# dtarb/TauDEM

Measured on AMD Instinct MI355X. Metric: Mcells/s (PitRemove->D8FlowDir->AreaD8 pipeline), higher is better.
Workload: dtype f32

## Files before the change

### taudem_amd/csrc/flats.hpp

```cpp
#pragma once
#include <algorithm>
#include <functional>
#include <vector>

#include "context.hpp"
#include "device_common.hpp"
#include "strips.hpp"
#include "tile_relax.hpp"

struct FlatLevels { int T; int Tr; int has_pits; };
struct FlatPhases { const char *classify, *levels, *stats, *directions, *next; };
static inline const FlatPhases& flat_phases(int iteration) {
    static const FlatPhases P[4] = {{"flats 1: classify", "flats 1: level fields", "flats 1: statistics", "flats 1: directions", "flats 1: next elev"},
                                    {"flats 2: classify", "flats 2: level fields", "flats 2: statistics", "flats 2: directions", "flats 2: next elev"},
                                    {"flats 3: classify", "flats 3: level fields", "flats 3: statistics", "flats 3: directions", "flats 3: next elev"},
                                    {"flats 4+: classify", "flats 4+: level fields", "flats 4+: statistics", "flats 4+: directions", "flats 4+: next elev"}};
    return P[iteration < 1 ? 0 : (iteration > 4 ? 3 : iteration - 1)];
}
using lvl_t = int16_t;
constexpr int LVL_SAT = 32767;
constexpr int TDX_FLATS_TOO_DEEP = -4242;
template <class LV>
struct FlatBuffersT { LV* lvl; LV* rq; };
using FlatBuffers = FlatBuffersT<lvl_t>;
// ... 291 lines not shown
    static __device__ __forceinline__ bool raw_can_move(S g) { return g >= 0; }
    __device__ __forceinline__ void store(size_t idx, int v) const { G[idx] = S(v); }
    __device__ __forceinline__ uint8_t cell_raw(size_t idx) const { return M[idx]; }
    static __device__ __forceinline__ void cell_decode(uint8_t m, int& cst, unsigned& mask) { cst = 0; mask = m; }
    static __device__ __forceinline__ int apply(int, int own, int m) {
        int t = m + INC;
        if (sizeof(S) == 2 && INC) t = unsigned(t - LVL_SAT) < unsigned(inf() - LVL_SAT) ? LVL_SAT : t;
        return t < own ? t : own;
    }
    static __device__ __forceinline__ int cell_floor(int cst, int) { return cst; }
    static __device__ __forceinline__ bool settled(int, int v) { return v <= 1; }
    static __device__ __forceinline__ int act_never() { return int(0x80000000u); }
    static __device__ __forceinline__ int act_threshold(uint8_t m, int v) { return m ? v - INC : act_never(); }
    static __device__ __forceinline__ int act_threshold_raw(S g) { return g >= 0 ? decode(g) - INC : act_never(); }

    __device__ __forceinline__ int macro_update(const tilek::TileGeom& g, int tile, int k, int* __restrict__ lds, tilek::TileLds& TL, uint32_t* __restrict__ flags_next,
                                                unsigned long long* __restrict__ dbg = nullptr) const {
        const int tid = int(threadIdx.x);
        const unsigned long long tq0 = dbg ? __builtin_readcyclecounter() : 0ull;
        const int W = k * tilek::TS, L = W + 2;
        const int tx0 = tile % g.tiles_x, ty0 = tile / g.tiles_x;
        const int X0 = tx0 * tilek::TS, Y0 = ty0 * tilek::TS;
        const size_t pitch = size_t(g.nx);
        int* const h = lds; int* const pre = h + MACRO_LMAX; int* const suf = pre + MACRO_LMAX; int* const pm = suf + MACRO_LMAX; int* const sp = pm + MACRO_LMAX;
        int* const acc = sp + MACRO_LMAX;
        int* const moved = acc + 4 * (MACRO_LMAX - 2);
        constexpr int AW = MACRO_LMAX - 2;
        if (tid < 8) moved[tid] = 0;
        __syncthreads();
        auto rim_idx = [&](int e, int i) -> size_t {
            const int x = e == 2 ? 0 : (e == 3 ? W - 1 : i), y = e == 0 ? 0 : (e == 1 ? W - 1 : i);
// ... 126 lines not shown
                    for (int i = j - 2; i <= j; i++) if (i >= 0 && i < W && chg[E * AW + i] < best) best = chg[E * AW + i];
                    gain = best + INC < decode(raw_ring[E][u]);
                }
                const int p = j == 0 ? -1 : (j - 1) / tilek::TS;
                const int p0 = __builtin_amdgcn_readfirstlane(p);
                const unsigned long long b_lo = __ballot(gain && p == p0), b_hi = __ballot(gain && p != p0);
                if ((tid & 63) == 0) {
                    if (b_lo != 0ull) atomicOr(&moved[E], 1 << (p0 + 1));
                    if (b_hi != 0ull) atomicOr(&moved[E], 1 << (p0 + 2));
                }
            }
        __syncthreads();
        const unsigned long long tq2 = dbg ? __builtin_readcyclecounter() : 0ull;
        if (tid < 4 * (k + 2)) {
            const int e = tid / (k + 2), j = tid % (k + 2) - 1;
            if (((moved[e] >> (j + 1)) & 1) && out_target >= 0) {
                if (atomicMax(&flags_next[tilek::entry_tile(uint32_t(out_target))], tilek::FLAG_HALO) == 0u) TL.pend[atomicAdd(&TL.npend, 1u)] = uint32_t(out_target);
            }
        }
        __syncthreads();
        if (dbg && tid == 0) {
            const unsigned long long tq3 = __builtin_readcyclecounter();
            atomicAdd(dbg + 9, tq1 - tq0); atomicAdd(dbg + 10, tq2 - tq1); atomicAdd(dbg + 11, tq3 - tq2);
        }
        return 0;
    }
};
using LevelOp = LevelOpT<1, lvl_t>;
using ReachOp = LevelOpT<0, int32_t>;

template <class LV>
static __global__ __launch_bounds__(256) void flat_stats_kernel(const uint32_t* __restrict__ list, unsigned long long nq,
                                                                const LV* __restrict__ lvl, const LV* __restrict__ rq,
// ... 292 lines not shown
    Op op{field, mask};
    if constexpr (Op::kHasPlain) op.TM = tile_masked;
    for (;;) {
        bool left = false;
        int rc = (st.multi() && eager_rounds > 0) ? tile_relax_run_bounded(ctx, op, geom, sc, eager_rounds, &left, rounds, launches) : tile_relax_run(ctx, op, geom, sc, rounds, launches);
        if (rc != TDX_OK) return rc;
        if (!st.multi()) return TDX_OK;
        int64_t changed = 0;
        rc = strip_exchange<typename Op::Raw>(ctx, st, field, typename Op::Raw(-1), sc.flags, geom.tiles_x, &changed, true, left ? 1 : 0);
        if (rc != TDX_OK) return rc;
        if (changed == 0) return TDX_OK;
    }
}

using StreamClassifyFn = std::function<void(const tilek::TileGeom&, uint8_t* fmask, uint8_t* rmask, uint32_t* tile_flags, uint8_t* tile_masked, uint8_t* notfull)>;
template <class Traits, class LV>
static int flats_bfs(tdx_context* ctx, Traits tr, const float* Z, const Strip& st, const uint32_t* qlist, unsigned long long nq,
                     FlatBuffersT<LV> b, FlatLevels* out, tdx_stats* stats, const StreamClassifyFn* stream_classify = nullptr, int iteration = 1) {
    using LOp = flatk::LevelOpT<1, LV>;
    const FlatPhases& ph = flat_phases(iteration);
    ctx->phase = ph.classify;
    hipStream_t s = ctx->stream;
    const int nx = st.nx;
    const size_t n = size_t(nx) * size_t(st.ny_arr);
    const tilek::TileGeom geom = tilek::make_geom(nx, st.ny_arr, st.y0, st.y1);
    const int ntiles = geom.tiles_x * geom.tiles_y;
    unsigned long long* d_cnt = reinterpret_cast<unsigned long long*>(ctx->d_mail);
    uint8_t* fmask = static_cast<uint8_t*>(ctx->scratch(TDX_S_E, n));
    uint8_t* rmask = static_cast<uint8_t*>(ctx->scratch(TDX_S_F, n));
    uint32_t* flags0 = static_cast<uint32_t*>(ctx->scratch(TDX_S_G, size_t(ntiles) * 4 * 2 + size_t(ntiles)));
// ... 49 lines not shown
    if (macro_k) {
        const int y_lo = st.multi() ? st.y0 + 1 : st.y0, y_hi = st.multi() ? st.y1 - 1 : st.y1;
        const unsigned nreg = unsigned(((geom.tiles_x + 7) / 8) * ((geom.tiles_y + 7) / 8));
        hipLaunchKernelGGL(flatk::find_blocks_kernel, dim3((nreg + 63) / 64, 2), dim3(64), 0, s, notfull, geom.tiles_x, geom.tiles_y, nx, y_lo, y_hi, macro_k, remapF, blkF, remapR, blkR);
        geomF.remap = remapF; geomF.blk_k = blkF;
        geomR.remap = remapR; geomR.blk_k = blkR;
    }
    if (pair) {
        uint32_t* listB = flagsB + ntiles;
        const bool two_streams = getenv("TDX_FLATS_FUSED") == nullptr || getenv("TDX_RELAX_LDS") != nullptr;
        const uint32_t* start_flags = two_streams ? flags0 : nullptr;
        if (!two_streams) {
            TDX_HIP_CHECK(ctx, hipMemcpyAsync(flags, flags0, size_t(ntiles) * 4, hipMemcpyDeviceToDevice, s));
            TDX_HIP_CHECK(ctx, hipMemcpyAsync(flagsB, flags0, size_t(ntiles) * 4, hipMemcpyDeviceToDevice, s));
        }
        for (;;) {
            rc = two_streams ? tile_relax_run_pair(ctx, LOp{b.lvl, fmask, tmask}, tilek::Sched{flags, list, counts},
                                                   LOp{b.rq, rmask, no_plain ? tmask : nullptr}, tilek::Sched{flagsB, listB, countsB}, geomF, &rounds_fall, &launches, start_flags, &geomR)
                             : tile_relax_run_fused(ctx, LOp{b.lvl, fmask, tmask}, tilek::Sched{flags, list, counts},
                                                    LOp{b.rq, rmask, no_plain ? tmask : nullptr}, tilek::Sched{flagsB, listB, countsB}, geom, &rounds_fall, &launches);
            if (rc != TDX_OK) return rc;
            start_flags = nullptr;
            if (!st.multi()) break;
            int64_t ch_fall = 0, ch_rise = 0;
            rc = strip_exchange<LV>(ctx, st, b.lvl, LV(-1), flags, geom.tiles_x, &ch_fall);
            if (rc != TDX_OK) return rc;
            rc = strip_exchange<LV>(ctx, st, b.rq, LV(-1), flagsB, geom.tiles_x, &ch_rise);
            if (rc != TDX_OK) return rc;
            int64_t changed = ch_fall + ch_rise;
            rc = strip_allreduce(ctx, st, &changed, 1, TDX_OP_SUM);
            if (rc != TDX_OK) return rc;
            if (changed == 0) break;
        }
    } else {
        const unsigned cg = tdx_blocks_for(size_t(ntiles), 256);
        TDX_HIP_CHECK(ctx, hipMemcpyAsync(flags, flags0, size_t(ntiles) * 4, hipMemcpyDeviceToDevice, s));
        if (macro_k) hipLaunchKernelGGL(flatk::block_flags_kernel, dim3(cg), dim3(256), 0, s, flags, remapF, ntiles);
// ... 61 lines not shown
```

### taudem_amd/csrc/pitremove.hip

```cpp
#include "context.hpp"
#include "device_common.hpp"
#include "strips.hpp"
#include "tile_relax.hpp"

namespace {

constexpr int SEED_ROWS = 16;
constexpr int SEED_CF = 8;
template <int MODE>
__global__ __launch_bounds__(256) void pit_seed_kernel(const float* __restrict__ Z, const int16_t* __restrict__ mask,
                                                       float* __restrict__ W, int nx, int ny, int y_own0, int y_own1, float nodata, int step,
                                                       float* __restrict__ Zc, float* __restrict__ Wc, int nxc, int nyc, int nbx, int xmap) {
    const int bx = tdxk::xcd_block_x(nbx, xmap);
    if (bx < 0) return;
    const int x = bx * 64 + (threadIdx.x & 63);
    const int ybase = y_own0 + blockIdx.y * (4 * SEED_ROWS) + (threadIdx.x >> 6) * SEED_ROWS;
    const bool colok = x < nx;
    const int xc = colok ? x : nx - 1, xm = xc > 0 ? xc - 1 : xc, xp = xc < nx - 1 ? xc + 1 : xc;
    const int lane = int(threadIdx.x & 63);
    const bool edge_lane = lane == 0 || lane == 63;
    const int xe = lane == 0 ? xm : xp;
    float zm[SEED_ROWS + 2], zedge[SEED_ROWS + 2];
#pragma unroll
    for (int j = 0; j < SEED_ROWS + 2; j++) {
// ... 189 lines not shown
};

}

static int pit_finish_level(tdx_context* ctx, const Strip& ls, float* Zc, float* Wc, int nxc, int nyc, int64_t cells_all, tilek::Sched sc, int depth,
                            int64_t* rounds, int64_t* launches, int64_t* own_rounds = nullptr);

static inline Strip pit_level_strip(const Strip& st, int nxc, int nyc) {
    Strip ls;
    ls.nx = nxc; ls.comm = st.comm;
    if (st.multi()) { ls.ny_arr = nyc + 2; ls.y0 = 1; ls.y1 = nyc + 1; ls.up = st.up; ls.down = st.down; }
    else { ls.ny_arr = nyc; ls.y0 = 0; ls.y1 = nyc; }
    return ls;
}

template <int NBR>
static int pit_relax_level(tdx_context* ctx, const Strip& ls, const float* Z, float* W, tilek::Sched sc, int64_t* rounds, int64_t* launches, int64_t* outer,
                           bool all_tiles = true) {
    const tilek::TileGeom g = tilek::make_geom(ls.nx, ls.ny_arr, ls.y0, ls.y1);
    for (;;) {
        int rc = tile_relax_run(ctx, PitOp<NBR>{Z, W}, g, sc, rounds, launches, all_tiles);
        all_tiles = false;
        if (rc != TDX_OK) return rc;
        if (outer) (*outer)++;
        if (!ls.multi()) break;
        int64_t changed = 0;
        rc = strip_exchange<float>(ctx, ls, W, TDX_FEL_NODATA, sc.flags, g.tiles_x, &changed, true);
        if (rc != TDX_OK) return rc;
        if (changed == 0) break;
    }
    return TDX_OK;
}

static int pit_coarse_start(tdx_context* ctx, const Strip& st, const float* Z, float* W, int nx, int nyo, int64_t cells_all, tilek::Sched sc, int depth,
                            int64_t* rounds, int64_t* launches) {
    if (depth >= 3 || cells_all < (int64_t(1) << 18) || nyo < 1) return TDX_OK;
// ... 76 lines not shown
            hipLaunchKernelGGL(pit_seed_kernel<2>, sgrid, dim3(256), 0, s, d_dem, d_mask, d_fel, st.nx, st.ny_arr, st.y0, st.y1, dem_nodata, 1, Zc + off, Wc + off, nxc, nyc, sbx, sxmap);
            if (stats) stats->launches[TDX_K_STENCIL]++;
        }
    } else {
        TdxSpan sp(ctx, TDX_K_STENCIL);
        hipLaunchKernelGGL(pit_seed_kernel<0>, sgrid, dim3(256), 0, s, d_dem, d_mask, d_fel, st.nx, st.ny_arr, st.y0, st.y1, dem_nodata, fourway ? 2 : 1,
                           static_cast<float*>(nullptr), static_cast<float*>(nullptr), 0, 0, sbx, sxmap);
        if (stats) stats->launches[TDX_K_STENCIL]++;
    }
    ctx->phase = "fine level";
    rc = strip_exchange<float>(ctx, st, d_fel, TDX_FEL_NODATA);
    if (rc != TDX_OK) return rc;
    {
        TdxSpan sp(ctx, TDX_K_RELAX);
        bool all_tiles = true;
        const int vc_env = getenv("TDX_PIT_VCYCLE_AFTER") ? std::max(0, atoi(getenv("TDX_PIT_VCYCLE_AFTER"))) : 8;
        if (used_coarse && vc_env > 0) {
            bool left = false;
            rc = tile_relax_run_bounded(ctx, PitOp<8>{d_dem, d_fel}, geom, sched, vc_env, &left, &rounds, &launches, true);
            if (rc != TDX_OK) return rc;
            all_tiles = false;
            const int vc_min = getenv("TDX_PIT_VCYCLE_MIN") ? atoi(getenv("TDX_PIT_VCYCLE_MIN")) : 16;
            if (st.multi() || (left && level1_rounds >= vc_min)) {
                const int nxc = (st.nx + CF - 1) / CF, nyc = (nyo + CF - 1) / CF;
                const Strip ls = pit_level_strip(st, nxc, nyc);
                const size_t off = size_t(ls.y0) * size_t(nxc);
                float* Zc = static_cast<float*>(ctx->scratch(TDX_S_D, size_t(nxc) * size_t(ls.ny_arr) * 4));
                float* Wc = static_cast<float*>(ctx->scratch(TDX_S_E, size_t(nxc) * size_t(ls.ny_arr) * 4));
                const tilek::TileGeom gc = tilek::make_geom(ls.nx, ls.ny_arr, ls.y0, ls.y1);
                const size_t ntc = size_t(gc.tiles_x) * size_t(gc.tiles_y);
                uint32_t* cflags = static_cast<uint32_t*>(ctx->scratch(TDX_S_L, ntc * 4 * (1 + tilek::SCHED_LIST_WORDS)));
                unsigned long long* ccounts = static_cast<unsigned long long*>(ctx->scratch(TDX_S_M, size_t(tilek::COUNT_RING) * 16));
                float* Ur = static_cast<float*>(ctx->scratch(TDX_S_N, size_t(nxc) * size_t(nyc) * 4));
                if (!Zc || !Wc || !cflags || !ccounts || !Ur) return TDX_ERR_NOMEM;
// ... 6 lines not shown
                    rc = strip_exchange<float>(ctx, ls, Wc, TDX_FEL_NODATA, cflags, gc.tiles_x, &changed);
                    if (rc != TDX_OK) return rc;
                }
                rc = pit_relax_level<8>(ctx, ls, Zc, Wc, tilek::Sched{cflags, cflags + ntc, ccounts}, &rounds, &launches, nullptr, false);
                if (rc != TDX_OK) return rc;
                hipLaunchKernelGGL(pit_prolong_min_kernel, dim3((st.nx + 63) / 64, (nyc + 3) / 4), dim3(256), 0, s, d_fel + size_t(st.y0) * size_t(st.nx), st.nx, nyo, Wc + off, Ur, nxc, nyc,
                                   st.y0, st.ny_arr, geom.tiles_x, flags);
                ctx->phase = "fine level";
                if (st.multi()) {
                    int64_t changed = 0;
                    rc = strip_exchange<float>(ctx, st, d_fel, TDX_FEL_NODATA, flags, geom.tiles_x, &changed);
                    if (rc != TDX_OK) return rc;
                }
            }
        }
        rc = fourway ? pit_relax_level<4>(ctx, st, d_dem, d_fel, sched, &rounds, &launches, &outer, all_tiles) : pit_relax_level<8>(ctx, st, d_dem, d_fel, sched, &rounds, &launches, &outer, all_tiles);
        if (rc != TDX_OK) return rc;
        if (stats) stats->launches[TDX_K_RELAX] += launches;
    }
    TDX_HIP_CHECK(ctx, hipGetLastError());
    if (stats) { stats->rounds = rounds; stats->cells_evaluated = outer; }
    ctx->end_call();
    return TDX_OK;
}

static int pitremove_check(tdx_context* ctx, const void* dem, const void* fel, int64_t nx, int64_t ny, int64_t halo, const char* who) {
    if (!ctx || !dem || !fel || nx <= 0 || ny <= 0) return tdx_fail(ctx, TDX_ERR_ARG, who);
    return too_big(nx, ny + halo) ? tdx_fail(ctx, TDX_ERR_ARG, "raster larger than 2^32 cells per device strip") : TDX_OK;
}

extern "C" int tdx_pitremove_dev(tdx_context* ctx, const float* d_dem, int64_t nx, int64_t ny, float dem_nodata,
// ... 22 lines not shown
```

### taudem_amd/csrc/tile_relax.hpp

```cpp
#pragma once
#include <atomic>
#include <algorithm>
#include <chrono>
#include <cstdlib>
#include <functional>
#include <type_traits>

#include "context.hpp"
#include "device_common.hpp"

namespace tilek {
using namespace tdxk;

constexpr int TS = 64;
constexpr int LH = TS + 2;
constexpr int LP = LH + 1;
constexpr int RPW = 16;
constexpr int NWAVE = TS / RPW;
constexpr int NTHR = NWAVE * 64;
constexpr int COUNT_RING = 1024;
constexpr int MAX_SWEEPS = 8;
constexpr int PULL_MAX = 64;
constexpr unsigned MACRO_DEAL_MAX = 4096;
constexpr unsigned MACRO_WGS_MIN = MACRO_DEAL_MAX / PULL_MAX;
// ... 58 lines not shown


__device__ __forceinline__ unsigned mask_at(const unsigned (&pk)[RPW / 4], int r) { return (pk[r >> 2] >> (8 * (r & 3))) & 0xFFu; }

struct TileLds {
    int rim;
    unsigned long long top[2][NWAVE], bot[2][NWAVE];
    unsigned any[2][NWAVE];
    unsigned rows[NWAVE];
    unsigned next;
    unsigned long long base;
    unsigned npend;
    int chain;
    uint32_t pulled[PULL_MAX];
    uint32_t pend[PULL_MAX * 9];
};

constexpr uint32_t FLAG_HALO = 1u, FLAG_FULL = 2u;
constexpr uint32_t TILE_IDX_MASK = 0x07ffffffu;
constexpr int TILE_BLK_SHIFT = 27;
__device__ __forceinline__ int entry_tile(uint32_t e) { return int(e & TILE_IDX_MASK); }
__device__ __forceinline__ int entry_blk_k(uint32_t e) { const unsigned c = (e >> TILE_BLK_SHIFT) & 3u; return c ? 1 << c : 0; }

__device__ __forceinline__ void activate_tiles_around(int x, int y, int nx, int ny, int tiles_x, uint32_t* __restrict__ tile_flags) {
#pragma unroll
    for (int dy = -1; dy <= 1; dy++)
#pragma unroll
        for (int dx = -1; dx <= 1; dx++) {
            const int xn = x + dx, yn = y + dy;
            if (xn >= 0 && xn < nx && yn >= 0 && yn < ny) tile_flags[(yn / TS) * tiles_x + xn / TS] = FLAG_FULL;
// ... 644 lines not shown
                    if (threadIdx.x == 0 && (bal == 0ull || (bal & (bal - 1ull)) != 0ull)) L.chain = -1;
                }
                __builtin_amdgcn_fence(__ATOMIC_SEQ_CST, "agent");
                __syncthreads();
                const int ch = L.chain;
                if (ch == -1) break;
                if (entry_blk_k(uint32_t(ch))) break;
                tile = entry_tile(uint32_t(ch));
                full = ch < 0;
            }
            if (res & (RES_CHANGED | RES_CAPPED)) flag_neighbours(res, tile, g, flags_next, L);
        }
    }
}

template <class Op, class = void>
struct relax_waves : std::integral_constant<int, 4> {};
template <class Op>
struct relax_waves<Op, std::void_t<decltype(Op::kWaves)>> : std::integral_constant<int, Op::kWaves> {};
template <class Body>
__device__ __forceinline__ void round_driver(const uint32_t* __restrict__ list, unsigned long long* __restrict__ count, uint32_t* __restrict__ flags_cur,
                                             uint32_t* __restrict__ flags_next, uint32_t* __restrict__ list_next, unsigned pull_max, const TileGeom& g,
                                             TileLds& L, Body body) {
    round_driver(list, count, flags_cur, flags_next, list_next, pull_max, g, L, body, blockIdx.x, gridDim.x);
}

template <class Op, class = void>
struct has_plain : std::false_type {};
template <class Op>
struct has_plain<Op, std::enable_if_t<Op::kHasPlain>> : std::true_type {};

template <class Op, class = void>
struct has_macro : std::false_type {};
template <class Op>
struct has_macro<Op, std::enable_if_t<(Op::kMacroLdsWords > 0)>> : std::true_type {};
template <class Op, bool = has_macro<Op>::value>
struct macro_lds_words : std::integral_constant<int, 0> {};
template <class Op>
struct macro_lds_words<Op, true> : std::integral_constant<int, Op::kMacroLdsWords> {};

template <class Op>
__device__ __forceinline__ void macro_role(const Op& op, const TileGeom& g, const uint32_t* __restrict__ list, unsigned long long* __restrict__ count,
                                           uint32_t* __restrict__ flags_next, uint32_t* __restrict__ list_next, int* __restrict__ lds, TileLds& L, unsigned bid, unsigned nblocks,
                                           unsigned long long* __restrict__ dbg) {
    const unsigned nact = unsigned(count[0]);
    if (threadIdx.x == 0) L.npend = 0u;
    auto serve = [&](unsigned nb) {
        for (unsigned b = 0; b < nb; b++) {
            const int tile = entry_tile(L.pulled[b]), kb = entry_blk_k(L.pulled[b]);
            const unsigned long long tc0 = dbg ? __builtin_readcyclecounter() : 0ull;
            (void)op.macro_update(g, tile, kb, lds, L, flags_next, dbg);
            if (dbg && threadIdx.x == 0) { atomicAdd(dbg + 13, __builtin_readcyclecounter() - tc0); atomicAdd(dbg + 14, 1ull); }
            const unsigned npend = L.npend;
            if (threadIdx.x == 0) L.base = npend ? atomicAdd(count + 1, (unsigned long long)npend) : 0ull;
            __syncthreads();
            const unsigned long long lb = L.base;
            for (unsigned q = threadIdx.x; q < npend; q += blockDim.x) list_next[lb + q] = L.pend[q];
            __syncthreads();
            if (threadIdx.x == 0) L.npend = 0u;
        }
    };
    if (nact <= MACRO_DEAL_MAX) {
        constexpr int PER = 16;
        static_assert(PER * NTHR == MACRO_DEAL_MAX, "every entry of a dealt round is looked at");
        uint32_t ent[PER];
        unsigned kk[PER];
        const unsigned first = threadIdx.x * PER;
        (void)first;
#pragma unroll
        for (int j = 0; j < PER; j++) { const unsigned i = unsigned(j) * NTHR + threadIdx.x; ent[j] = i < nact ? list[i] : 0u; }
        unsigned mine = 0;
#pragma unroll
        for (int j = 0; j < PER; j++) { kk[j] = unsigned(entry_blk_k(ent[j])); mine += kk[j] != 0u; }
        unsigned incl = mine;
// ... 32 lines not shown
        serve(nb);
    }
}

template <class Op, bool REG>
__global__ __launch_bounds__(NTHR, relax_waves<Op>::value) void relax_kernel(Op op, TileGeom g, const uint32_t* __restrict__ list, unsigned long long* __restrict__ count,
                                                    uint32_t* __restrict__ flags_cur, uint32_t* __restrict__ flags_next,
                                                    uint32_t* __restrict__ list_next, unsigned pull_max, unsigned long long* __restrict__ dbg, unsigned grid_tiles) {
    using T = typename Op::T;
    static_assert(sizeof(T) == 4, "tile engine works on 4-byte values");
    constexpr int kLdsWords = REG ? (REG_LDS_WORDS > macro_lds_words<Op>::value ? REG_LDS_WORDS : macro_lds_words<Op>::value) : LH * LP;
    __shared__ T sV[kLdsWords];
    __shared__ TileLds L;
    if constexpr (REG && has_macro<Op>::value) {
        if (grid_tiles != 0u && blockIdx.x >= grid_tiles) {
            macro_role(op, g, list, count, flags_next, list_next, reinterpret_cast<int*>(sV), L, blockIdx.x - grid_tiles, gridDim.x - grid_tiles, dbg);
            return;
        }
    }
    const unsigned nblocks = grid_tiles != 0u ? grid_tiles : gridDim.x;
    round_driver(list, count, flags_cur, flags_next, list_next, pull_max, g, L, [&](int tile, bool full) {
        if constexpr (REG && has_plain<Op>::value) {
            if (!__builtin_amdgcn_readfirstlane(int(op.tile_masked(tile)))) return relax_tile_reg(op.plain(), g, tile, sV, L, dbg);
        }
        return REG ? relax_tile_reg(op, g, tile, sV, L, dbg) : relax_tile(op, g, tile, full, sV, L, dbg);
    }, blockIdx.x, nblocks);
}

struct RoundArgs { const uint32_t* list; unsigned long long* count; uint32_t* flags_cur; uint32_t* flags_next; uint32_t* list_next; };
template <class Op>
__global__ __launch_bounds__(NTHR, relax_waves<Op>::value) void relax_pair_kernel(Op opA, Op opB, TileGeom g, RoundArgs a, RoundArgs b, unsigned gridA,
                                                                                  unsigned pull_max) {
    using T = typename Op::T;
    static_assert(sizeof(T) == 4, "tile engine works on 4-byte values");
    __shared__ T sV[REG_LDS_WORDS];
    __shared__ TileLds L;
    const bool second = blockIdx.x >= gridA;
    const Op op = second ? opB : opA;
    const RoundArgs ra = second ? b : a;
    round_driver(ra.list, ra.count, ra.flags_cur, ra.flags_next, ra.list_next, pull_max, g, L,
                 [&](int tile, bool) {
// ... 147 lines not shown
    const int t = blockIdx.x * 256 + threadIdx.x;
    const uint32_t f = t < ntiles ? flags0[t] : 0u;
    const uint32_t ra = (remapA != nullptr && t < ntiles) ? remapA[t] : uint32_t(t), rb = (remapB != nullptr && t < ntiles) ? remapB[t] : uint32_t(t);
    const uint32_t fa = entry_tile(ra) != t ? 0u : f, fb = entry_tile(rb) != t ? 0u : f;
    if (t < ntiles) { flagsA[t] = fa; flagsB[t] = fb; flagsA1[t] = 0u; flagsB1[t] = 0u; }
    const unsigned long long pa = block_reserve(fa != 0u ? 1u : 0u, countA);
    if (fa != 0u) listA[pa] = ra;
    const unsigned long long pb = block_reserve(fb != 0u ? 1u : 0u, countB);
    if (fb != 0u) listB[pb] = rb;
}
static __global__ __launch_bounds__(256) void all_start_kernel(int ntiles, uint32_t* __restrict__ flags, uint32_t* __restrict__ flags1, uint32_t* __restrict__ list,
                                                               unsigned long long* __restrict__ counts) {
    const int t = blockIdx.x * 256 + threadIdx.x;
    if (t < ntiles) { flags[t] = FLAG_FULL; flags1[t] = 0u; list[t] = uint32_t(t); }
    if (t < 2 * COUNT_RING) counts[t] = t == 0 ? (unsigned long long)ntiles : 0ull;
}

static __global__ __launch_bounds__(256) void ring_wrap_kernel(unsigned long long* __restrict__ counts, int r) {
    const unsigned long long pending = counts[r];
    __syncthreads();
    for (int i = threadIdx.x; i < 2 * COUNT_RING; i += 256) counts[i] = 0ull;
    __syncthreads();
    if (threadIdx.x == 0) counts[0] = pending;
}

static __global__ __launch_bounds__(256) void flags_fold_kernel(uint32_t* __restrict__ f_first, uint32_t* __restrict__ f_second, int ntiles) {
    const int t = blockIdx.x * 256 + threadIdx.x;
    if (t >= ntiles) return;
    const uint32_t b = f_second[t];
    if (b) { f_second[t] = 0u; if (b > f_first[t]) f_first[t] = b; }
// ... 42 lines not shown
    const unsigned err = unsigned(host_mail[3] & 0xffffffffull);
    *gave_up = err != 0;
    if (err) {
        fprintf(stderr, "taudem_amd: asynchronous tile worklist gave up (code %u, head %llu tail %llu pending %d); continuing with the round schedule\n", err,
                (unsigned long long)host_mail[0], (unsigned long long)host_mail[1], int(host_mail[2] & 0xffffffffull));
        hipLaunchKernelGGL(fill_u32_kernel, dim3(cgrid), dim3(256), 0, s, sc.flags, FLAG_FULL, size_t(ntiles));
    }
    return TDX_OK;
}

template <class Op>
struct RoundRunner {
    tdx_context* ctx; hipStream_t s; Op op; tilek::TileGeom g; tilek::Sched sc; uint64_t* h; unsigned long long* dbg;
    int ntiles; unsigned cgrid, grid_full, grid_small;
    bool print_counts = false;
    int ring_len;
    bool lds_variant;
    unsigned pull_max;
    int r = 0, parity = 0, batch = 4;
    int r_enq = 0, parity_enq = 0, n_enq = 0, n_col = 0, fl_batch[2] = {0, 0};
    bool polled[2] = {false, false};
    uint64_t fl_tag[2] = {0, 0};
    int ev_base = 0;
    int batch_max = 64;
    bool done = false;
    int64_t rounds = 0, launches = 0;
    bool short_tail = getenv("TDX_RELAX_LONG_TAIL") == nullptr;
    unsigned long long last_count = 0;
    std::function<void(const tilek::TileGeom& rg, unsigned grid, hipStream_t st, const uint32_t* list, unsigned long long* count, uint32_t* flags_cur,
                       uint32_t* flags_next, uint32_t* list_next, unsigned pull_max)> custom_launch;
    RoundRunner(tdx_context* c, hipStream_t st, Op o, tilek::TileGeom geom, tilek::Sched sched, uint64_t* host_mail, unsigned long long* d)
        : ctx(c), s(st), op(o), g(geom), sc(sched), h(host_mail), dbg(d) {
        ntiles = g.tiles_x * g.tiles_y;
        cgrid = tdx_blocks_for(size_t(ntiles), 256);
        grid_full = unsigned(std::min(ntiles, 8 * ctx->num_cus));
        static const int gs_env = getenv("TDX_RELAX_GRID_SMALL") ? std::max(1, atoi(getenv("TDX_RELAX_GRID_SMALL"))) : 0;
        grid_small = unsigned(std::min(ntiles, gs_env ? gs_env : ctx->num_cus));
        const char* e = getenv("TDX_RELAX_RING");
        ring_len = e ? std::max(3, std::min(atoi(e), tilek::COUNT_RING)) : tilek::COUNT_RING;
        lds_variant = getenv("TDX_RELAX_LDS") != nullptr;
        const char* pm = getenv("TDX_RELAX_PULL");
        pull_max = pm ? unsigned(std::max(1, std::min(atoi(pm), tilek::PULL_MAX))) : 16u;
    }
    uint32_t* list_of(int p) const { return sc.list + size_t(p) * size_t(ntiles); }
    uint32_t* flags_of(int p) const { return p ? sc.list + 2 * size_t(ntiles) : sc.flags; }
    bool prestarted = false;
    bool all_tiles = false;
    int start() {
        using namespace tilek;
        r = 0; parity = 0;
        r_enq = 0; parity_enq = 0; n_enq = 0; n_col = 0;
        if (prestarted) return TDX_OK;
        if (all_tiles) {
            hipLaunchKernelGGL(all_start_kernel, dim3(tdx_blocks_for(size_t(std::max(ntiles, 2 * COUNT_RING)), 256)), dim3(256), 0, s, ntiles, sc.flags, flags_of(1), list_of(0), sc.counts);
            return TDX_OK;
        }
        TDX_HIP_CHECK(ctx, hipMemsetAsync(sc.counts, 0, size_t(2 * COUNT_RING) * sizeof(unsigned long long), s));
        TDX_HIP_CHECK(ctx, hipMemsetAsync(flags_of(1), 0, size_t(ntiles) * 4, s));
        hipLaunchKernelGGL(first_list_kernel, dim3(cgrid), dim3(256), 0, s, sc.flags, ntiles, list_of(0), sc.counts, g.remap);
        r = 0; parity = 0;
        r_enq = 0; parity_enq = 0; n_enq = 0; n_col = 0;
        return TDX_OK;
    }
// ... 78 lines not shown
                    return tdx_fail(ctx, TDX_ERR_HIP, "tile schedule: no report from a batch of rounds after " + std::to_string(int(limit_s)) + " s");
            }
            __builtin_ia32_pause();
        }
        std::atomic_thread_fence(std::memory_order_acquire);
        return TDX_OK;
    }
    void collect() {
        const int slot = n_col & 1, nb = fl_batch[slot];
        const volatile uint64_t* hs = h + slot * TDX_MAIL_RUN_SLOT;
        for (int b = 0; b < nb; b++) {
            const uint64_t cnt = polled[slot] ? (hs[b] & 0xffffffffull) : hs[b];
            if (cnt == 0) { done = true; break; }
            last_count = cnt;
            rounds++;
            if (print_counts) fprintf(stderr, " %llu", (unsigned long long)cnt);
        }
        r += nb;
        parity = (parity + nb) & 1;
        n_col++;
    }
    static int pipelined_batch_max() {
        static const int v = getenv("TDX_RELAX_BATCH") ? std::max(2, std::min(atoi(getenv("TDX_RELAX_BATCH")), 64)) : 16;
        return v;
    }
    int drive() {
        batch_max = pipelined_batch_max();
        int rc = start();
        if (rc != TDX_OK) return rc;
        rc = enqueue();
        if (rc != TDX_OK) return rc;
// ... 62 lines not shown
    while (!A.done || !B.done) {
        rc = enqueue_fused(A, B);
        if (rc != TDX_OK) return rc;
        rc = A.wait_oldest();
        if (rc != TDX_OK) return rc;
        if (!A.done) A.collect(); else A.n_col++;
        if (!B.done) B.collect(); else B.n_col++;
    }
    if (rounds_out) *rounds_out += A.rounds + B.rounds;
    if (launches_out) *launches_out += A.launches;
    return TDX_OK;
}

template <class Op>
static int tile_relax_run_pair(tdx_context* ctx, Op opA, tilek::Sched scA, Op opB, tilek::Sched scB, tilek::TileGeom g, int64_t* rounds_out,
                               int64_t* launches_out, const uint32_t* flags0 = nullptr, const tilek::TileGeom* gB = nullptr) {
    if (flags0) {
        const int ntiles = g.tiles_x * g.tiles_y;
        hipLaunchKernelGGL(tilek::pair_start_kernel, dim3(tdx_blocks_for(size_t(ntiles), 256)), dim3(256), 0, ctx->stream, flags0, ntiles, scA.flags, scA.list + 2 * size_t(ntiles),
                           scA.list, scA.counts, scB.flags, scB.list + 2 * size_t(ntiles), scB.list, scB.counts, g.remap, gB ? gB->remap : g.remap);
    }
    if (!ctx->stream2) {
        TDX_HIP_CHECK(ctx, hipStreamCreateWithFlags(&ctx->stream2, hipStreamNonBlocking));
        TDX_HIP_CHECK(ctx, hipEventCreateWithFlags(&ctx->ev_fork, hipEventDisableTiming));
    }
    TDX_HIP_CHECK(ctx, hipEventRecord(ctx->ev_fork, ctx->stream));
    TDX_HIP_CHECK(ctx, hipStreamWaitEvent(ctx->stream2, ctx->ev_fork, 0));
    RoundRunner<Op> A(ctx, ctx->stream, opA, g, scA, ctx->h_mail + TDX_MAIL_RUN_A, nullptr), B(ctx, ctx->stream2, opB, gB ? *gB : g, scB, ctx->h_mail + TDX_MAIL_RUN_B, nullptr);
    B.ev_base = 2;
    A.prestarted = B.prestarted = flags0 != nullptr;
    A.batch_max = B.batch_max = RoundRunner<Op>::pipelined_batch_max();
    int rc = A.start();
    if (rc != TDX_OK) return rc;
    rc = B.start();
    if (rc != TDX_OK) return rc;
    rc = A.enqueue();
    if (rc != TDX_OK) return rc;
    rc = B.enqueue();
    if (rc != TDX_OK) return rc;
    while (!A.done || !B.done) {
        if (!A.done) { rc = A.enqueue(); if (rc != TDX_OK) return rc; }
        if (!B.done) { rc = B.enqueue(); if (rc != TDX_OK) return rc; }
        if (!A.done) { rc = A.wait_oldest(); if (rc != TDX_OK) return rc; A.collect(); }
        if (!B.done) { rc = B.wait_oldest(); if (rc != TDX_OK) return rc; B.collect(); }
    }
    TDX_HIP_CHECK(ctx, hipEventRecord(ctx->ev_fork, ctx->stream2));
    TDX_HIP_CHECK(ctx, hipStreamWaitEvent(ctx->stream, ctx->ev_fork, 0));
    if (rounds_out) *rounds_out += A.rounds + B.rounds;
    if (launches_out) *launches_out += A.launches + B.launches;
    return TDX_OK;
}

template <class Op>
static int tile_relax_run_bounded(tdx_context* ctx, Op op, tilek::TileGeom g, tilek::Sched sc, int max_rounds, bool* active_left, int64_t* rounds_out,
                                  int64_t* launches_out, bool all_tiles = false) {
    RoundRunner<Op> run(ctx, ctx->stream, op, g, sc, ctx->h_mail + TDX_MAIL_RUN_A, nullptr);
    run.all_tiles = all_tiles;
    run.batch = run.batch_max = std::max(2, std::min(max_rounds, 64));
    static const int debug_level = getenv("TDX_DEBUG_ROUNDS") ? atoi(getenv("TDX_DEBUG_ROUNDS")) : 0;
    run.print_counts = debug_level > 0;
    if (debug_level == 2) fprintf(stderr, "\nrounds(%d tiles, at most %d):", run.ntiles, max_rounds);
    *active_left = false;
    int rc = run.start();
    if (rc != TDX_OK) return rc;
    while (!run.done) {
        rc = run.enqueue();
        if (rc != TDX_OK) return rc;
        rc = run.wait_oldest();
        if (rc != TDX_OK) return rc;
        run.collect();
        if (!run.done && run.rounds >= max_rounds) { *active_left = true; break; }
    }
    if (*active_left && run.parity)
        hipLaunchKernelGGL(tilek::flags_fold_kernel, dim3(tdx_blocks_for(size_t(run.ntiles), 256)), dim3(256), 0, ctx->stream, run.flags_of(0), run.flags_of(1), run.ntiles);
    if (rounds_out) *rounds_out += run.rounds;
    if (launches_out) *launches_out += run.launches;
    return TDX_OK;
}

template <class Op>
static int tile_relax_run(tdx_context* ctx, Op op, tilek::TileGeom g, tilek::Sched sc, int64_t* rounds_out, int64_t* launches_out, bool all_tiles = false) {
    using namespace tilek;
    hipStream_t s = ctx->stream;
    const int ntiles = g.tiles_x * g.tiles_y;
    static const int debug_level = getenv("TDX_DEBUG_ROUNDS") ? atoi(getenv("TDX_DEBUG_ROUNDS")) : 0;
    static const bool debug = debug_level == 1;
    static const bool force_rounds = getenv("TDX_RELAX_ASYNC") == nullptr;
    unsigned long long* dbg = nullptr;
    if (debug) {
        dbg = reinterpret_cast<unsigned long long*>(ctx->d_mail) + TDX_MAIL_DBG_RELAX;
        TDX_HIP_CHECK(ctx, hipMemsetAsync(dbg, 0, 128, s));
    }
    int64_t rounds = 0, launches = 0;
    bool need_rounds = force_rounds;
    if (!force_rounds) {
        bool gave_up = false;
        int rc = tile_relax_async_finish(ctx, s, op, g, sc, TDX_S_Q, ctx->h_mail, dbg, &gave_up);
        if (rc != TDX_OK) return rc;
        launches += 1;
        rounds += 1;
        need_rounds = gave_up;
    }
    if (need_rounds) {
        RoundRunner<Op> run(ctx, s, op, g, sc, ctx->h_mail + TDX_MAIL_RUN_A, dbg);
        run.all_tiles = all_tiles && force_rounds;
        run.print_counts = debug_level > 0;
        if (debug_level == 2) fprintf(stderr, "\nrounds(%d tiles):", ntiles);
        int rc = run.drive();
        if (rc != TDX_OK) return rc;
        rounds += run.rounds;
        launches += run.launches;
    }
    if (debug) {
        TDX_HIP_CHECK(ctx, hipMemcpyAsync(ctx->h_mail, dbg, 128, hipMemcpyDeviceToHost, s));
        TDX_HIP_CHECK(ctx, hipStreamSynchronize(s));
        fprintf(stderr, "tile_relax_run(%d tiles, %s): %lld rounds, %llu tile activations, %llu sweeps; queue pops %llu pushes %llu activations %llu\n", ntiles,
                need_rounds ? "rounds" : "worklist", (long long)rounds, (unsigned long long)ctx->h_mail[1], (unsigned long long)ctx->h_mail[0],
                (unsigned long long)ctx->h_mail[2], (unsigned long long)ctx->h_mail[3], (unsigned long long)ctx->h_mail[4]);
        const double na = double(ctx->h_mail[1] ? ctx->h_mail[1] : 1);
        fprintf(stderr, "    cycles per activation (s_memtime): load %.0f, sweeps %.0f, write-back %.0f\n", double(ctx->h_mail[6]) / na, double(ctx->h_mail[7]) / na,
                double(ctx->h_mail[8]) / na);
// ... 11 lines not shown
```

Baseline: 12550.

## Add four-colour Gauss-Seidel tile relaxation rounds for PitRemove start

Introduces a coloured relaxation mode in which the tile worklist is split by a 2x2 tile colouring and each round runs four launches, one per colour. Activations of higher-numbered colours go into the current round, so a change can travel across several tiles within one round, as in Gauss-Seidel. PitRemove enables two coloured rounds by default at the start. The flats path gets the hook with a default of zero. This aims to cut the number of rounds needed for propagation, at the cost of four times as many kernel launches per coloured round and a list-splitting pass.

```diff
diff --git a/taudem_amd/csrc/flats.hpp b/taudem_amd/csrc/flats.hpp
--- a/taudem_amd/csrc/flats.hpp
+++ b/taudem_amd/csrc/flats.hpp
@@ -329,7 +329,8 @@
     static __device__ __forceinline__ int act_threshold(uint8_t m, int v) { return m ? v - INC : act_never(); }
     static __device__ __forceinline__ int act_threshold_raw(S g) { return g >= 0 ? decode(g) - INC : act_never(); }
 
-    __device__ __forceinline__ int macro_update(const tilek::TileGeom& g, int tile, int k, int* __restrict__ lds, tilek::TileLds& TL, uint32_t* __restrict__ flags_next,
+    template <class Sink>
+    __device__ __forceinline__ int macro_update(const tilek::TileGeom& g, int tile, int k, int* __restrict__ lds, tilek::TileLds& TL, const Sink& sink,
                                                 unsigned long long* __restrict__ dbg = nullptr) const {
         const int tid = int(threadIdx.x);
         const unsigned long long tq0 = dbg ? __builtin_readcyclecounter() : 0ull;
@@ -486,9 +487,7 @@
         const unsigned long long tq2 = dbg ? __builtin_readcyclecounter() : 0ull;
         if (tid < 4 * (k + 2)) {
             const int e = tid / (k + 2), j = tid % (k + 2) - 1;
-            if (((moved[e] >> (j + 1)) & 1) && out_target >= 0) {
-                if (atomicMax(&flags_next[tilek::entry_tile(uint32_t(out_target))], tilek::FLAG_HALO) == 0u) TL.pend[atomicAdd(&TL.npend, 1u)] = uint32_t(out_target);
-            }
+            if (((moved[e] >> (j + 1)) & 1) && out_target >= 0) sink.raise(out_target, tilek::FLAG_HALO, TL);
         }
         __syncthreads();
         if (dbg && tid == 0) {
@@ -811,6 +810,7 @@
 }
 
 using StreamClassifyFn = std::function<void(const tilek::TileGeom&, uint8_t* fmask, uint8_t* rmask, uint32_t* tile_flags, uint8_t* tile_masked, uint8_t* notfull)>;
+constexpr int FLATS_COLOURED_ROUNDS = 0;
 template <class Traits, class LV>
 static int flats_bfs(tdx_context* ctx, Traits tr, const float* Z, const Strip& st, const uint32_t* qlist, unsigned long long nq,
                      FlatBuffersT<LV> b, FlatLevels* out, tdx_stats* stats, const StreamClassifyFn* stream_classify = nullptr, int iteration = 1) {
@@ -890,13 +890,16 @@
             TDX_HIP_CHECK(ctx, hipMemcpyAsync(flags, flags0, size_t(ntiles) * 4, hipMemcpyDeviceToDevice, s));
             TDX_HIP_CHECK(ctx, hipMemcpyAsync(flagsB, flags0, size_t(ntiles) * 4, hipMemcpyDeviceToDevice, s));
         }
+        int coloured = (iteration == 1 && two_streams && getenv("TDX_RELAX_LDS") == nullptr) ? tilek::coloured_rounds(FLATS_COLOURED_ROUNDS, "TDX_RELAX_COLOURED_FLATS") : 0;
         for (;;) {
             rc = two_streams ? tile_relax_run_pair(ctx, LOp{b.lvl, fmask, tmask}, tilek::Sched{flags, list, counts},
-                                                   LOp{b.rq, rmask, no_plain ? tmask : nullptr}, tilek::Sched{flagsB, listB, countsB}, geomF, &rounds_fall, &launches, start_flags, &geomR)
+                                                   LOp{b.rq, rmask, no_plain ? tmask : nullptr}, tilek::Sched{flagsB, listB, countsB}, geomF, &rounds_fall, &launches, start_flags, &geomR,
+                                                   coloured)
                              : tile_relax_run_fused(ctx, LOp{b.lvl, fmask, tmask}, tilek::Sched{flags, list, counts},
                                                     LOp{b.rq, rmask, no_plain ? tmask : nullptr}, tilek::Sched{flagsB, listB, countsB}, geom, &rounds_fall, &launches);
             if (rc != TDX_OK) return rc;
             start_flags = nullptr;
+            coloured = 0;
             if (!st.multi()) break;
             int64_t ch_fall = 0, ch_rise = 0;
             rc = strip_exchange<LV>(ctx, st, b.lvl, LV(-1), flags, geom.tiles_x, &ch_fall);
diff --git a/taudem_amd/csrc/pitremove.hip b/taudem_amd/csrc/pitremove.hip
--- a/taudem_amd/csrc/pitremove.hip
+++ b/taudem_amd/csrc/pitremove.hip
@@ -227,12 +227,13 @@
     return ls;
 }
 
+constexpr int PIT_COLOURED_ROUNDS = 2;
 template <int NBR>
 static int pit_relax_level(tdx_context* ctx, const Strip& ls, const float* Z, float* W, tilek::Sched sc, int64_t* rounds, int64_t* launches, int64_t* outer,
-                           bool all_tiles = true) {
+                           bool all_tiles = true, int coloured = 0) {
     const tilek::TileGeom g = tilek::make_geom(ls.nx, ls.ny_arr, ls.y0, ls.y1);
     for (;;) {
-        int rc = tile_relax_run(ctx, PitOp<NBR>{Z, W}, g, sc, rounds, launches, all_tiles);
+        int rc = tile_relax_run(ctx, PitOp<NBR>{Z, W}, g, sc, rounds, launches, all_tiles, all_tiles ? coloured : 0);
         all_tiles = false;
         if (rc != TDX_OK) return rc;
         if (outer) (*outer)++;
@@ -339,10 +340,11 @@
     {
         TdxSpan sp(ctx, TDX_K_RELAX);
         bool all_tiles = true;
+        const int coloured = tilek::coloured_rounds(PIT_COLOURED_ROUNDS, "TDX_RELAX_COLOURED_PIT");
         const int vc_env = getenv("TDX_PIT_VCYCLE_AFTER") ? std::max(0, atoi(getenv("TDX_PIT_VCYCLE_AFTER"))) : 8;
         if (used_coarse && vc_env > 0) {
             bool left = false;
-            rc = tile_relax_run_bounded(ctx, PitOp<8>{d_dem, d_fel}, geom, sched, vc_env, &left, &rounds, &launches, true);
+            rc = tile_relax_run_bounded(ctx, PitOp<8>{d_dem, d_fel}, geom, sched, vc_env, &left, &rounds, &launches, true, coloured);
             if (rc != TDX_OK) return rc;
             all_tiles = false;
             const int vc_min = getenv("TDX_PIT_VCYCLE_MIN") ? atoi(getenv("TDX_PIT_VCYCLE_MIN")) : 16;
@@ -379,7 +381,7 @@
                 }
             }
         }
-        rc = fourway ? pit_relax_level<4>(ctx, st, d_dem, d_fel, sched, &rounds, &launches, &outer, all_tiles) : pit_relax_level<8>(ctx, st, d_dem, d_fel, sched, &rounds, &launches, &outer, all_tiles);
+        rc = fourway ? pit_relax_level<4>(ctx, st, d_dem, d_fel, sched, &rounds, &launches, &outer, all_tiles, coloured) : pit_relax_level<8>(ctx, st, d_dem, d_fel, sched, &rounds, &launches, &outer, all_tiles, coloured);
         if (rc != TDX_OK) return rc;
         if (stats) stats->launches[TDX_K_RELAX] += launches;
     }
diff --git a/taudem_amd/csrc/tile_relax.hpp b/taudem_amd/csrc/tile_relax.hpp
--- a/taudem_amd/csrc/tile_relax.hpp
+++ b/taudem_amd/csrc/tile_relax.hpp
@@ -4,6 +4,7 @@
 #include <chrono>
 #include <cstdlib>
 #include <functional>
+#include <string>
 #include <type_traits>
 
 #include "context.hpp"
@@ -96,6 +97,8 @@
     int chain;
     uint32_t pulled[PULL_MAX];
     uint32_t pend[PULL_MAX * 9];
+    unsigned npk[4];
+    unsigned long long basek[4];
 };
 
 constexpr uint32_t FLAG_HALO = 1u, FLAG_FULL = 2u;
@@ -770,6 +773,101 @@
     }
 }
 
+struct PlainSink {
+    uint32_t* flags_next; uint32_t* list_next; unsigned long long* count_next;
+    __device__ __forceinline__ void init(TileLds& L) const { if (threadIdx.x == 0) L.npend = 0u; }
+    __device__ __forceinline__ void raise(int target, uint32_t flag, TileLds& L) const {
+        if (atomicMax(&flags_next[entry_tile(uint32_t(target))], flag) == 0u) L.pend[atomicAdd(&L.npend, 1u)] = uint32_t(target);
+    }
+    __device__ __forceinline__ void flush(TileLds& L) const {
+        const unsigned npend = L.npend;
+        if (threadIdx.x == 0) L.base = npend ? atomicAdd(count_next, (unsigned long long)npend) : 0ull;
+        __syncthreads();
+        const unsigned long long lb = L.base;
+        for (unsigned q = threadIdx.x; q < npend; q += blockDim.x) list_next[lb + q] = L.pend[q];
+        __syncthreads();
+        if (threadIdx.x == 0) L.npend = 0u;
+    }
+};
+
+constexpr int COLOUR_PULL_MAX = 16;
+constexpr int COLOUR_PEND = COLOUR_PULL_MAX * 9;
+static_assert(4 * COLOUR_PEND <= PULL_MAX * 9, "four colour regions in TileLds::pend");
+struct ColourRound {
+    const uint32_t* list; unsigned long long* count;
+    uint32_t* list_cur; unsigned long long* cnt_cur;
+    uint32_t* list_nxt; unsigned long long* cnt_nxt;
+    uint32_t* flags_cur; uint32_t* flags_next;
+    unsigned off[4];
+    int colour, last, tiles_x;
+};
+__device__ __forceinline__ int tile_colour(int tile, int tiles_x) { return ((tile % tiles_x) & 1) | (((tile / tiles_x) & 1) << 1); }
+struct ColourSink {
+    const ColourRound& cr;
+    __device__ __forceinline__ void init(TileLds& L) const { if (threadIdx.x < 4) L.npk[threadIdx.x] = 0u; }
+    __device__ __forceinline__ void raise(int target, uint32_t flag, TileLds& L) const {
+        const int t = entry_tile(uint32_t(target)), k = tile_colour(t, cr.tiles_x);
+        uint32_t* f = k > cr.colour ? cr.flags_cur : cr.flags_next;
+        if (atomicMax(&f[t], flag) == 0u) L.pend[k * COLOUR_PEND + int(atomicAdd(&L.npk[k], 1u))] = uint32_t(target);
+    }
+    __device__ __forceinline__ void flush(TileLds& L) const {
+        if (threadIdx.x < 4) {
+            const unsigned k = threadIdx.x, n = L.npk[k];
+            unsigned long long* c = int(k) > cr.colour ? cr.cnt_cur + k : (cr.last ? cr.cnt_nxt : cr.cnt_nxt + k);
+            L.basek[k] = n ? atomicAdd(c, (unsigned long long)n) : 0ull;
+        }
+        __syncthreads();
+#pragma unroll
+        for (int k = 0; k < 4; k++) {
+            const unsigned n = L.npk[k];
+            uint32_t* dst = k > cr.colour ? cr.list_cur + cr.off[k] : (cr.last ? cr.list_nxt : cr.list_nxt + cr.off[k]);
+            const unsigned long long lb = L.basek[k];
+            for (unsigned q = threadIdx.x; q < n; q += blockDim.x) dst[lb + q] = L.pend[k * COLOUR_PEND + int(q)];
+        }
+        __syncthreads();
+        if (threadIdx.x < 4) L.npk[threadIdx.x] = 0u;
+    }
+};
+template <class Body>
+__device__ __forceinline__ void colour_round_driver(const ColourRound& cr, unsigned pull_max, const TileGeom& g, TileLds& L, Body body, unsigned bid, unsigned nblocks) {
+    const ColourSink sink{cr};
+    const unsigned nact = unsigned(cr.count[0]);
+    unsigned long long* cursor = cr.count + COUNT_RING;
+    unsigned pull = nact / (2u * nblocks);
+    pull_max = pull_max > unsigned(COLOUR_PULL_MAX) ? unsigned(COLOUR_PULL_MAX) : pull_max;
+    pull = pull < 1u ? 1u : (pull > pull_max ? pull_max : pull);
+    if (bid * pull >= nact) return;
+    sink.init(L);
+    for (;;) {
+        __syncthreads();
+        sink.flush(L);
+        if (threadIdx.x == 0) L.next = unsigned(atomicAdd(cursor, (unsigned long long)pull));
+        __syncthreads();
+        const unsigned first = L.next;
+        if (first >= nact) break;
+        const unsigned last = first + pull < nact ? first + pull : nact;
+        if (threadIdx.x < last - first) L.pulled[threadIdx.x] = cr.list[first + threadIdx.x];
+        __syncthreads();
+        for (unsigned it = first; it < last; it++) {
+            const uint32_t ent = L.pulled[it - first];
+            const int tile = entry_tile(ent);
+            const bool full = cr.flags_cur[tile] >= FLAG_FULL;
+            if (entry_blk_k(ent)) {
+                __syncthreads();
+                if (threadIdx.x == 0) cr.flags_cur[tile] = 0u;
+                continue;
+            }
+            const int res = body(tile, full);
+            if (threadIdx.x == 0) cr.flags_cur[tile] = 0u;
+            if (res & (RES_CHANGED | RES_CAPPED)) {
+                uint32_t flag;
+                const int target = activation_target(res, tile, g, &flag);
+                if (target >= 0) sink.raise(target, flag, L);
+            }
+        }
+    }
+}
+
 template <class Op, class = void>
 struct relax_waves : std::integral_constant<int, 4> {};
 template <class Op>
@@ -795,25 +893,19 @@
 template <class Op>
 struct macro_lds_words<Op, true> : std::integral_constant<int, Op::kMacroLdsWords> {};
 
-template <class Op>
-__device__ __forceinline__ void macro_role(const Op& op, const TileGeom& g, const uint32_t* __restrict__ list, unsigned long long* __restrict__ count,
-                                           uint32_t* __restrict__ flags_next, uint32_t* __restrict__ list_next, int* __restrict__ lds, TileLds& L, unsigned bid, unsigned nblocks,
+template <class Op, class Sink>
+__device__ __forceinline__ void macro_role(const Op& op, const TileGeom& g, const uint32_t* __restrict__ list, const unsigned long long* __restrict__ count,
+                                           const Sink& sink, int* __restrict__ lds, TileLds& L, unsigned bid, unsigned nblocks,
                                            unsigned long long* __restrict__ dbg) {
     const unsigned nact = unsigned(count[0]);
-    if (threadIdx.x == 0) L.npend = 0u;
+    sink.init(L);
     auto serve = [&](unsigned nb) {
         for (unsigned b = 0; b < nb; b++) {
             const int tile = entry_tile(L.pulled[b]), kb = entry_blk_k(L.pulled[b]);
             const unsigned long long tc0 = dbg ? __builtin_readcyclecounter() : 0ull;
-            (void)op.macro_update(g, tile, kb, lds, L, flags_next, dbg);
+            (void)op.macro_update(g, tile, kb, lds, L, sink, dbg);
             if (dbg && threadIdx.x == 0) { atomicAdd(dbg + 13, __builtin_readcyclecounter() - tc0); atomicAdd(dbg + 14, 1ull); }
-            const unsigned npend = L.npend;
-            if (threadIdx.x == 0) L.base = npend ? atomicAdd(count + 1, (unsigned long long)npend) : 0ull;
-            __syncthreads();
-            const unsigned long long lb = L.base;
-            for (unsigned q = threadIdx.x; q < npend; q += blockDim.x) list_next[lb + q] = L.pend[q];
-            __syncthreads();
-            if (threadIdx.x == 0) L.npend = 0u;
+            sink.flush(L);
         }
     };
     if (nact <= MACRO_DEAL_MAX) {
@@ -876,7 +968,7 @@
     __shared__ TileLds L;
     if constexpr (REG && has_macro<Op>::value) {
         if (grid_tiles != 0u && blockIdx.x >= grid_tiles) {
-            macro_role(op, g, list, count, flags_next, list_next, reinterpret_cast<int*>(sV), L, blockIdx.x - grid_tiles, gridDim.x - grid_tiles, dbg);
+            macro_role(op, g, list, count, PlainSink{flags_next, list_next, count + 1}, reinterpret_cast<int*>(sV), L, blockIdx.x - grid_tiles, gridDim.x - grid_tiles, dbg);
             return;
         }
     }
@@ -887,6 +979,28 @@
         }
         return REG ? relax_tile_reg(op, g, tile, sV, L, dbg) : relax_tile(op, g, tile, full, sV, L, dbg);
     }, blockIdx.x, nblocks);
+}
+
+template <class Op>
+__global__ __launch_bounds__(NTHR, relax_waves<Op>::value) void relax_colour_kernel(Op op, TileGeom g, ColourRound cr, unsigned pull_max, unsigned long long* __restrict__ dbg,
+                                                                                    unsigned grid_tiles) {
+    using T = typename Op::T;
+    static_assert(sizeof(T) == 4, "tile engine works on 4-byte values");
+    constexpr int kLdsWords = REG_LDS_WORDS > macro_lds_words<Op>::value ? REG_LDS_WORDS : macro_lds_words<Op>::value;
+    __shared__ T sV[kLdsWords];
+    __shared__ TileLds L;
+    if constexpr (has_macro<Op>::value) {
+        if (grid_tiles != 0u && blockIdx.x >= grid_tiles) {
+            macro_role(op, g, cr.list, cr.count, ColourSink{cr}, reinterpret_cast<int*>(sV), L, blockIdx.x - grid_tiles, gridDim.x - grid_tiles, dbg);
+            return;
+        }
+    }
+    colour_round_driver(cr, pull_max, g, L, [&](int tile, bool) {
+        if constexpr (has_plain<Op>::value) {
+            if (!__builtin_amdgcn_readfirstlane(int(op.tile_masked(tile)))) return relax_tile_reg(op.plain(), g, tile, sV, L, dbg);
+        }
+        return relax_tile_reg(op, g, tile, sV, L, dbg);
+    }, blockIdx.x, grid_tiles != 0u ? grid_tiles : gridDim.x);
 }
 
 struct RoundArgs { const uint32_t* list; unsigned long long* count; uint32_t* flags_cur; uint32_t* flags_next; uint32_t* list_next; };
@@ -1064,6 +1178,27 @@
     const int t = blockIdx.x * 256 + threadIdx.x;
     if (t < ntiles) { flags[t] = FLAG_FULL; flags1[t] = 0u; list[t] = uint32_t(t); }
     if (t < 2 * COUNT_RING) counts[t] = t == 0 ? (unsigned long long)ntiles : 0ull;
+}
+
+constexpr int COLOUR_COUNT0 = 4;
+constexpr int COLOUR_MAX_ROUNDS = 16;
+struct ColourOff { unsigned o[4]; };
+static inline int coloured_rounds(int dflt, const char* own) {
+    const char* e = getenv(own);
+    if (!e) e = getenv("TDX_RELAX_COLOURED");
+    return e ? std::max(0, std::min(atoi(e), COLOUR_MAX_ROUNDS)) : dflt;
+}
+static __global__ __launch_bounds__(256) void colour_split_kernel(const uint32_t* __restrict__ list, unsigned long long* __restrict__ counts, int tiles_x, uint32_t* __restrict__ out,
+                                                                  ColourOff off) {
+    const unsigned i = blockIdx.x * 256u + threadIdx.x;
+    const bool on = i < unsigned(counts[0]);
+    const uint32_t e = on ? list[i] : 0u;
+    const int k = on ? tile_colour(entry_tile(e), tiles_x) : -1;
+#pragma unroll
+    for (int c = 0; c < 4; c++) {
+        const unsigned long long pos = block_reserve(k == c ? 1u : 0u, counts + COLOUR_COUNT0 + c);
+        if (k == c) out[off.o[c] + pos] = e;
+    }
 }
 
 static __global__ __launch_bounds__(256) void ring_wrap_kernel(unsigned long long* __restrict__ counts, int r) {
@@ -1136,6 +1271,7 @@
     tdx_context* ctx; hipStream_t s; Op op; tilek::TileGeom g; tilek::Sched sc; uint64_t* h; unsigned long long* dbg;
     int ntiles; unsigned cgrid, grid_full, grid_small;
     bool print_counts = false;
+    std::string* count_log = nullptr;
     int ring_len;
     bool lds_variant;
     unsigned pull_max;
@@ -1164,11 +1300,65 @@
         const char* pm = getenv("TDX_RELAX_PULL");
         pull_max = pm ? unsigned(std::max(1, std::min(atoi(pm), tilek::PULL_MAX))) : 16u;
     }
-    uint32_t* list_of(int p) const { return sc.list + size_t(p) * size_t(ntiles); }
+    int coloured = 0;
+    int list_flip = 0;
+    uint32_t* list_of(int p) const { return sc.list + size_t(p ^ list_flip) * size_t(ntiles); }
     uint32_t* flags_of(int p) const { return p ? sc.list + 2 * size_t(ntiles) : sc.flags; }
     bool prestarted = false;
     bool all_tiles = false;
     int start() {
+        list_flip = 0;
+        int rc = start_plain();
+        if (rc != TDX_OK || coloured <= 0 || lds_variant || custom_launch) return rc;
+        return start_coloured();
+    }
+    int start_coloured() {
+        using namespace tilek;
+        const int R = std::min(coloured, COLOUR_MAX_ROUNDS);
+        const unsigned cx[2] = {unsigned(g.tiles_x + 1) / 2u, unsigned(g.tiles_x) / 2u}, cy[2] = {unsigned(g.tiles_y + 1) / 2u, unsigned(g.tiles_y) / 2u};
+        ColourOff off;
+        off.o[0] = 0u; off.o[1] = cx[0] * cy[0]; off.o[2] = off.o[1] + cx[1] * cy[0]; off.o[3] = off.o[2] + cx[0] * cy[1];
+        hipLaunchKernelGGL(colour_split_kernel, dim3(cgrid), dim3(256), 0, s, list_of(0), sc.counts, g.tiles_x, list_of(1), off);
+        list_flip = 1;
+        TileGeom cg = g;
+        cg.cnt_host = nullptr; cg.cnt_dev = nullptr; cg.cnt_tag = 0ull;
+        static const int macro_wgs = getenv("TDX_MACRO_WGS") ? std::max(1, atoi(getenv("TDX_MACRO_WGS"))) : 4;
+        const unsigned gm = (has_macro<Op>::value && g.blk_k != nullptr) ? std::max(unsigned(macro_wgs * ctx->num_cus), MACRO_WGS_MIN) : 0u;
+        const bool timed = ctx->kernel_timing && s == ctx->stream;
+        for (int j = 0; j < R; j++) {
+            const int p = j & 1;
+            ColourRound cr;
+            cr.list_cur = list_of(p); cr.cnt_cur = sc.counts + COLOUR_COUNT0 + 4 * j;
+            cr.list_nxt = list_of(p ^ 1); cr.cnt_nxt = sc.counts + COLOUR_COUNT0 + 4 * (j + 1);
+            cr.flags_cur = flags_of(p); cr.flags_next = flags_of(p ^ 1);
+            for (int k = 0; k < 4; k++) cr.off[k] = off.o[k];
+            cr.last = j == R - 1; cr.tiles_x = g.tiles_x;
+            for (int c = 0; c < 4; c++) {
+                cr.colour = c; cr.list = cr.list_cur + off.o[c]; cr.count = cr.cnt_cur + c;
+                const unsigned gmc = c == 0 ? gm : 0u;
+                const int sp = timed ? ctx->span_begin(TDX_K_TILEK) : -1;
+                hipLaunchKernelGGL((relax_colour_kernel<Op>), dim3(grid_full + gmc), dim3(NTHR), 0, s, op, cg, cr, pull_max, dbg, gmc ? grid_full : 0u);
+                ctx->span_end(sp);
+                if (timed && ctx->cur_stats) ctx->cur_stats->launches[TDX_K_TILEK]++;
+            }
+        }
+        if (print_counts) {
+            unsigned long long hc[4 * COLOUR_MAX_ROUNDS];
+            TDX_HIP_CHECK(ctx, hipStreamSynchronize(s));
+            TDX_HIP_CHECK(ctx, hipMemcpy(hc, sc.counts + COLOUR_COUNT0, size_t(4 * R) * sizeof(unsigned long long), hipMemcpyDeviceToHost));
+            for (int j = 0; j < R; j++) {
+                char buf[160];
+                snprintf(buf, sizeof buf, " %llu[%llu+%llu+%llu+%llu]", hc[4 * j] + hc[4 * j + 1] + hc[4 * j + 2] + hc[4 * j + 3], hc[4 * j], hc[4 * j + 1], hc[4 * j + 2], hc[4 * j + 3]);
+                if (count_log) *count_log += buf; else fputs(buf, stderr);
+            }
+        }
+        r = r_enq = COLOUR_COUNT0 + 4 * R;
+        parity = parity_enq = R & 1;
+        rounds += R; launches += 4 * R + 1;
+        last_count = (unsigned long long)ntiles;
+        return TDX_OK;
+    }
+    int start_plain() {
         using namespace tilek;
         r = 0; parity = 0;
         r_enq = 0; parity_enq = 0; n_enq = 0; n_col = 0;
@@ -1277,7 +1467,9 @@
             if (cnt == 0) { done = true; break; }
             last_count = cnt;
             rounds++;
-            if (print_counts) fprintf(stderr, " %llu", (unsigned long long)cnt);
+            if (print_counts) {
+                if (count_log) *count_log += " " + std::to_string((unsigned long long)cnt); else fprintf(stderr, " %llu", (unsigned long long)cnt);
+            }
         }
         r += nb;
         parity = (parity + nb) & 1;
@@ -1370,7 +1562,7 @@
 
 template <class Op>
 static int tile_relax_run_pair(tdx_context* ctx, Op opA, tilek::Sched scA, Op opB, tilek::Sched scB, tilek::TileGeom g, int64_t* rounds_out,
-                               int64_t* launches_out, const uint32_t* flags0 = nullptr, const tilek::TileGeom* gB = nullptr) {
+                               int64_t* launches_out, const uint32_t* flags0 = nullptr, const tilek::TileGeom* gB = nullptr, int coloured = 0) {
     if (flags0) {
         const int ntiles = g.tiles_x * g.tiles_y;
         hipLaunchKernelGGL(tilek::pair_start_kernel, dim3(tdx_blocks_for(size_t(ntiles), 256)), dim3(256), 0, ctx->stream, flags0, ntiles, scA.flags, scA.list + 2 * size_t(ntiles),
@@ -1385,6 +1577,10 @@
     RoundRunner<Op> A(ctx, ctx->stream, opA, g, scA, ctx->h_mail + TDX_MAIL_RUN_A, nullptr), B(ctx, ctx->stream2, opB, gB ? *gB : g, scB, ctx->h_mail + TDX_MAIL_RUN_B, nullptr);
     B.ev_base = 2;
     A.prestarted = B.prestarted = flags0 != nullptr;
+    A.coloured = B.coloured = coloured;
+    static const int debug_level = getenv("TDX_DEBUG_ROUNDS") ? atoi(getenv("TDX_DEBUG_ROUNDS")) : 0;
+    std::string logA, logB;
+    if (debug_level > 0) { A.print_counts = B.print_counts = true; A.count_log = &logA; B.count_log = &logB; }
     A.batch_max = B.batch_max = RoundRunner<Op>::pipelined_batch_max();
     int rc = A.start();
     if (rc != TDX_OK) return rc;
@@ -1402,6 +1598,7 @@
     }
     TDX_HIP_CHECK(ctx, hipEventRecord(ctx->ev_fork, ctx->stream2));
     TDX_HIP_CHECK(ctx, hipStreamWaitEvent(ctx->stream, ctx->ev_fork, 0));
+    if (debug_level > 0) fprintf(stderr, "\nrounds(pair, %d tiles) first field:%s\nrounds(pair, %d tiles) second field:%s", A.ntiles, logA.c_str(), B.ntiles, logB.c_str());
     if (rounds_out) *rounds_out += A.rounds + B.rounds;
     if (launches_out) *launches_out += A.launches + B.launches;
     return TDX_OK;
@@ -1409,9 +1606,10 @@
 
 template <class Op>
 static int tile_relax_run_bounded(tdx_context* ctx, Op op, tilek::TileGeom g, tilek::Sched sc, int max_rounds, bool* active_left, int64_t* rounds_out,
-                                  int64_t* launches_out, bool all_tiles = false) {
+                                  int64_t* launches_out, bool all_tiles = false, int coloured = 0) {
     RoundRunner<Op> run(ctx, ctx->stream, op, g, sc, ctx->h_mail + TDX_MAIL_RUN_A, nullptr);
     run.all_tiles = all_tiles;
+    run.coloured = coloured;
     run.batch = run.batch_max = std::max(2, std::min(max_rounds, 64));
     static const int debug_level = getenv("TDX_DEBUG_ROUNDS") ? atoi(getenv("TDX_DEBUG_ROUNDS")) : 0;
     run.print_counts = debug_level > 0;
@@ -1435,7 +1633,7 @@
 }
 
 template <class Op>
-static int tile_relax_run(tdx_context* ctx, Op op, tilek::TileGeom g, tilek::Sched sc, int64_t* rounds_out, int64_t* launches_out, bool all_tiles = false) {
+static int tile_relax_run(tdx_context* ctx, Op op, tilek::TileGeom g, tilek::Sched sc, int64_t* rounds_out, int64_t* launches_out, bool all_tiles = false, int coloured = 0) {
     using namespace tilek;
     hipStream_t s = ctx->stream;
     const int ntiles = g.tiles_x * g.tiles_y;
@@ -1461,6 +1659,7 @@
         RoundRunner<Op> run(ctx, s, op, g, sc, ctx->h_mail + TDX_MAIL_RUN_A, dbg);
         run.all_tiles = all_tiles && force_rounds;
         run.print_counts = debug_level > 0;
+        run.coloured = coloured;
         if (debug_level == 2) fprintf(stderr, "\nrounds(%d tiles):", ntiles);
         int rc = run.drive();
         if (rc != TDX_OK) return rc;
```

New measurement: 12590, median of 6. No clear change (+0.3%).
